# ajbrock/Neural-Photo-Editor

Hardware: NVIDIA H100
Metric: 64x64 images/sec IAN encode->decode @ batch 256 (higher is better)
Workload: dtype f32 (3-pass bf16 split on wgmma, fp32 accumulate)

## Files before the change

### neural-photo-editor_b200/csrc/ian_api.cu

```cuda
#include <cuda_runtime.h>

#include <algorithm>
#include <cmath>
#include <cstdarg>
#include <cstdio>
#include <cstdlib>
#include <cstring>
#include <map>
#include <string>
#include <vector>

#include <cuda.h>

#include "../../include/ian_b200.h"
#include "edge.h"
#include "tapgemm.h"

using namespace ian;

namespace {

thread_local std::string g_create_error;

inline uint16_t f2bf(float f) {
// ... 133 lines not shown
                                    "jvp_full_dec_fc2", "jvp_full_dec_conv1", "jvp_dec_conv2a", "jvp_dec_conv2a2", "jvp_full_dec_conv2",
                                    "jvp_dec_conv3a", "jvp_dec_conv3a2", "jvp_full_dec_conv3", "jvp_dec_conv4a", "jvp_dec_conv4a2",
                                    "jvp_full_dec_conv4", "rgb_head_jvp",
                                    "jvp_enc_conv2", "jvp_enc_conv3", "jvp_enc_conv4", "jvp_enc_fc1", "jvp_enc_head",
                                    "enc_conv1", "dec_out", "brush_seed", "enc_conv1_bwd",
                                    "wgrad_l_dec_fc2", "wgrad_dec_conv1", "wgrad_dec_conv2", "wgrad_dec_conv3", "wgrad_dec_out",
                                    "dec_out_jvp", "jvp_enc_conv1"};

struct DevWeights {
  __nv_bfloat16* b = nullptr;
  long long plane = 0;
  int ntiles = 0, Cout = 0, Cin = 0;
  float* scale = nullptr;
  float* shift = nullptr;
};

struct Plan;

}

struct ian_handle {
  int device = 0;
  int model_kind = 0;
  int path = IAN_PATH_TC;
  int passes = 3;
  float* sk_ws = nullptr;
  int* sk_flags = nullptr;
  int sk_epoch = 0;
  int streamk = 1;
  bool splitk = true;
  bool coop_finalize = true;
  bool pdl = true;
  bool graphs = true;
  bool capturing = false;
  bool finalized = false;
  cudaStream_t stream = nullptr;
  cudaStream_t h2d_stream = nullptr, d2h_stream = nullptr;
  std::vector<void*> host_allocs;
  int gw = 0, grank = 0, gn = 0, gcur = 0, gepoch = 0;
  float* gbuf = nullptr;
  float* gpeer_buf[8] = {nullptr};
  bool gconnected = false;
  float** gather_dsts = nullptr;
  int gather_ndst = 0;
  cudaStream_t push_stream = nullptr;
  cudaEvent_t g_comp[2] = {nullptr, nullptr}, g_done[2] = {nullptr, nullptr};
  bool g_done_valid[2] = {false, false};
  int g_last = -1;
  int push_ctas = 32;
  int push_mode = 0;
  void* train_ws = nullptr;
  size_t train_ws_bytes = 0;
  long long tickets = 0;
  struct Ticket { int id = -1, n = 0, slot = 0; };
  Ticket inflight[2];
  std::string err;
  int64_t launches = 0;
  std::map<std::string, HostParam> params;
  DevWeights w[L_COUNT];
  float* conv1_wt = nullptr;
  float* conv1_b = nullptr;
  __nv_bfloat16* conv1_tc_wt = nullptr;
  Conv1Maps* conv1_maps = nullptr;
  float* decout_wt = nullptr;
  float* conv1_bwd_wt = nullptr;
  __nv_bfloat16* conv1_bwd_tc_wt = nullptr;
// ... 480 lines not shown
int get_plan(ian_handle* h, int n, Plan** out) {
  auto it = h->plans.find(n);
  if (it != h->plans.end()) { *out = it->second; return IAN_OK; }
  Plan* pl = nullptr;
  int rc = build_plan(h, n, &pl);
  if (rc != IAN_OK) { if (pl) free_plan(pl); return rc; }
  h->plans[n] = pl;
  *out = pl;
  return IAN_OK;
}

struct ScopedTimer {
  ian_handle* h; int slot; cudaStream_t st; ian_handle::Timed tm{}; bool on;
  ScopedTimer(ian_handle* h_, int slot_, cudaStream_t st_) : h(h_), slot(slot_), st(st_), on(h_->timing) {
    if (on) { cudaEventCreate(&tm.e0); cudaEventCreate(&tm.e1); cudaEventRecord(tm.e0, st); }
  }
  ~ScopedTimer() {
    if (on) { cudaEventRecord(tm.e1, st); h->timed[slot].push_back(tm); }
  }
};

constexpr int kGraphMaxBatch = 32;

int run_gemm(ian_handle* h, Plan* pl, int l, cudaStream_t st) {
  TapGemm g = pl->g[l];
  if (g.ksplit < 1) return fail(h, IAN_ERR_INVALID, "layer %s is not part of this plan", kLayerNames[l]);
  g.passes = h->passes;
  g.out_t_bf16 = (g.out_f32_t && h->passes == 1) ? 1 : 0;
  const bool sk_ok = !h->capturing && (h->streamk == 2 || pl->n > kGraphMaxBatch);
  g.sk_ws = (h->streamk && sk_ok) ? h->sk_ws : nullptr;
  g.sk_force = h->streamk == 2 ? 1 : 0;
  g.sk_flags = h->sk_flags;
  g.sk_epoch = ++h->sk_epoch;
  ian_handle::Timed tm{};
  if (h->timing) {
    CUDA_TRY(h, cudaEventCreate(&tm.e0));
    CUDA_TRY(h, cudaEventCreate(&tm.e1));
  }
  if (h->path == IAN_PATH_SIMT) {
    g.ksplit = 1;
    g.ws = nullptr;
    if (h->timing) CUDA_TRY(h, cudaEventRecord(tm.e0, st));
    LAUNCH_TRY(h, launch_tapgemm_simt(g, st));
    if (h->timing) CUDA_TRY(h, cudaEventRecord(tm.e1, st));
  } else {
    if (h->timing) CUDA_TRY(h, cudaEventRecord(tm.e0, st));
    LAUNCH_TRY(h, launch_tapgemm_tc(g, pl->maps[l], st));
    if (h->timing) CUDA_TRY(h, cudaEventRecord(tm.e1, st));
    if (g.ksplit > 1) LAUNCH_TRY(h, launch_splitk_finalize(g, st));
  }
  if (h->timing) h->timed[l].push_back(tm);
  return IAN_OK;
}

int run_encode(ian_handle* h, Plan* pl, const float* x, const float* eps, float* z, cudaStream_t st, float* z_pre = nullptr) {
  const int n = pl->n;
  {
    ScopedTimer tm(h, T_CONV1, st);
    if (h->path == IAN_PATH_TC)
      LAUNCH_TRY(h, launch_conv1_tc(h->conv1_maps, pl->conv1_out, x, h->conv1_b, n, st));
    else
      LAUNCH_TRY(h, launch_conv1(x, h->conv1_wt, h->conv1_b, pl->a1.p, pl->a1.plane, n, st));
  }
  int rc;
  for (int l : kEncoder)
    if ((rc = run_gemm(h, pl, l, st)) != IAN_OK) return rc;
// ... 1333 lines not shown

extern "C" {

int ian_create(int model_kind, int device, ian_handle** out) {
  if (!out) return fail(nullptr, IAN_ERR_INVALID, "out is NULL");
  if (model_kind != IAN_MODEL_SIMPLE && model_kind != IAN_MODEL_FULL && model_kind != IAN_MODEL_V1)
    return fail(nullptr, IAN_ERR_UNSUPPORTED, "unknown model kind %d", model_kind);
  int ndev = 0;
  cudaError_t e = cudaGetDeviceCount(&ndev);
  if (e != cudaSuccess || ndev == 0)
    return fail(nullptr, IAN_ERR_CUDA, "no CUDA device: %s (this library has no CPU path)", cudaGetErrorString(e));
  if (device < 0 || device >= ndev) return fail(nullptr, IAN_ERR_INVALID, "device %d out of range [0,%d)", device, ndev);
  cudaDeviceProp prop;
  cudaGetDeviceProperties(&prop, device);
  if (prop.major != 9 || prop.minor != 0)
    return fail(nullptr, IAN_ERR_UNSUPPORTED, "device %d is sm_%d%d; libian_b200 is built for sm_90a only", device, prop.major, prop.minor);
  ian_handle* h = new ian_handle();
  h->device = device;
  h->model_kind = model_kind;
  DeviceGuard dg(device);
  if (cudaStreamCreateWithFlags(&h->stream, cudaStreamNonBlocking) != cudaSuccess ||
      cudaStreamCreateWithFlags(&h->h2d_stream, cudaStreamNonBlocking) != cudaSuccess ||
      cudaStreamCreateWithFlags(&h->d2h_stream, cudaStreamNonBlocking) != cudaSuccess) {
    delete h;
    return fail(nullptr, IAN_ERR_CUDA, "cudaStreamCreate failed");
  }
  if (const char* c = getenv("IAN_CHUNK")) { int v = atoi(c); if (v > 0) h->max_chunk = v > 4096 ? 4096 : v; }
  if (const char* c = getenv("IAN_PATH")) { if (!strcmp(c, "simt")) h->path = IAN_PATH_SIMT; }
  if (const char* c = getenv("IAN_STREAMK")) { const int v = atoi(c); h->streamk = v < 0 ? 0 : v > 2 ? 2 : v; }
  if (const char* c = getenv("IAN_SPLITK")) h->splitk = atoi(c) != 0;
  if (const char* c = getenv("IAN_PDL")) h->pdl = atoi(c) != 0;
  if (const char* c = getenv("IAN_FINALIZE8")) h->coop_finalize = atoi(c) != 0;
  if (const char* c = getenv("IAN_GRAPHS")) h->graphs = atoi(c) != 0;
  *out = h;
  return IAN_OK;
}

int ian_set_param(ian_handle* h, const char* name, const float* data, const int64_t* shape, int ndim) {
  if (!h || !name || !data || !shape) return fail(h, IAN_ERR_INVALID, "NULL argument");
  if (h->finalized) return fail(h, IAN_ERR_STATE, "model already finalized");
  int64_t elems = 0;
  int rc = check_param_shape(h, name, shape, ndim, &elems);
  if (rc != IAN_OK) return rc;
  HostParam& p = h->params[name];
  p.shape.assign(shape, shape + ndim);
  p.data.assign(data, data + elems);
  return IAN_OK;
}

int ian_set_made_ordering(ian_handle* h, const int32_t* ordering, int n) {
  if (!h || !ordering) return fail(h, IAN_ERR_INVALID, "NULL argument");
  if (h->finalized) return fail(h, IAN_ERR_STATE, "model already finalized");
  if (n != 100) return fail(h, IAN_ERR_INVALID, "ordering must have 100 entries (got %d)", n);
  std::vector<char> seen(100, 0);
  for (int i = 0; i < n; ++i) {
    if (ordering[i] < 0 || ordering[i] >= 100 || seen[ordering[i]]) return fail(h, IAN_ERR_INVALID, "ordering is not a permutation of 0..99");
    seen[ordering[i]] = 1;
  }
  h->made_ordering.assign(ordering, ordering + n);
  return IAN_OK;
}

int ian_model_param_count(int model_kind) {
  if (model_kind < 0 || model_kind > 2) return IAN_ERR_INVALID;
  return (int)cached_specs(model_kind).size();
}
// ... 574 lines not shown
```

### neural-photo-editor_b200/csrc/tapgemm.h

```cpp
#pragma once
#include <cuda_bf16.h>
#include <cuda_runtime.h>
#include <stdint.h>

#include <atomic>

namespace ian {

enum Act : int { ACT_NONE = 0, ACT_LRELU = 1, ACT_RELU = 2, ACT_ELU = 3, ACT_MASK = 4 };

constexpr int kMaxDevices = 64;
inline int cur_device() {
  int d = 0;
  cudaGetDevice(&d);
  return (d >= 0 && d < kMaxDevices) ? d : 0;
}
struct DeviceOnce {
  std::atomic<bool> done[kMaxDevices];
  bool is_done(int dev) const { return done[dev].load(std::memory_order_acquire); }
  void set_done(int dev) { done[dev].store(true, std::memory_order_release); }
};

inline bool& pdl_flag() {
  static thread_local bool on = false;
// ... 44 lines not shown
  int Hg, Wg;
  const __nv_bfloat16* b;
  long long b_plane;
  int Cout;
  int nphase;
  Phase phase[kMaxPhases];
  Tap taps[kMaxTaps];
  const float* scale;
  const float* shift;
  int scale_pix_stride;
  int act;
  const __nv_bfloat16* mask;
  float mask_slope;
  int res_after;
  __nv_bfloat16* out;
  long long out_plane;
  float* out_f32;
  int Hout, Wout, osh, osw;
  int ksplit;
  float* ws;
  long long ws_slab;
  const __nv_bfloat16* res;
  long long res_plane;
  __nv_bfloat16* out_raw;
  long long out_raw_plane;
  float* out_f32_t;
  int cout_real;
  int out_t_bf16;
  int passes;
  float* sk_ws;
  int* sk_flags;
  int sk_epoch;
  int sk_force;
};

__host__ __device__ inline void tile_shape(int Hg, int Wg, int& Wt, int& Ht, int& Nt) {
  Wt = Wg < 128 ? Wg : 128;
  Ht = Hg < 128 / Wt ? Hg : 128 / Wt;
  Nt = 128 / (Wt * Ht);
}

__device__ __forceinline__ float act_apply(float v, int act) {
  switch (act) {
    case ACT_LRELU: return 0.6f * v + 0.4f * fabsf(v);
    case ACT_RELU:  return 0.5f * (v + fabsf(v));
    case ACT_ELU:   return v > 0.f ? v : expm1f(v);
    default:        return v;
  }
}

__device__ __forceinline__ void split_bf16(float v, __nv_bfloat16& hi, __nv_bfloat16& lo) {
  hi = __float2bfloat16_rn(v);
  lo = __float2bfloat16_rn(v - __bfloat162float(hi));
}

int launch_tapgemm_simt(const TapGemm& g, cudaStream_t st);
struct TcMaps;
TcMaps* tc_build_maps(const TapGemm& g, char* err, int errlen);
void tc_free_maps(TcMaps*);
int launch_tapgemm_tc(const TapGemm& g, const TcMaps* maps, cudaStream_t st);
int launch_splitk_finalize(const TapGemm& g, cudaStream_t st);
int tc_tile_width(const TcMaps* maps);
int tc_num_sms();
size_t tc_sk_workspace_floats();
size_t tc_sk_flag_ints();

// ... 21 lines not shown
```

### neural-photo-editor_b200/csrc/tapgemm_tc.cu

```cuda
#include <cuda.h>

#include <cstdio>
#include <cstring>
#include <vector>

#include "tapgemm.h"
#include "tc_ptx.cuh"

namespace ian {

struct TcMaps {
  CUtensorMap a[4];
  CUtensorMap b;
  CUtensorMap a1[4];
  CUtensorMap b1;
  int Wt, Ht, Nt, BN;
  mutable int sk_choice;
};

namespace {

using namespace tc;

constexpr int BM = 128;
constexpr int BK = 64;

constexpr int kEpiWarps = 8;
constexpr int kThreadsCta = 32 * kEpiWarps + 32;

template <int BN, int PASSES> struct TcCfg {
  static constexpr int kPlanes = PASSES == 3 ? 2 : 1;
  static constexpr int kATileBytes = BM * BK * 2 * kPlanes;
  static constexpr int kBTileBytes = BN * BK * 2 * kPlanes;
  static constexpr int kStageBytes = kATileBytes + kBTileBytes;
  static constexpr int kRound = (PASSES == 3 && BN > 32) ? 32 : BN;
  static constexpr int kRounds = BN / kRound;
  static constexpr int kLd = kRound + 8;
  static constexpr int kStagingBytes = BM * kLd * 4;
  static constexpr int kStageSmem = kEpiWarps * 1024;
  static constexpr int kStagesFit = (220 * 1024 - kStagingBytes - kStageSmem) / kStageBytes;
  static constexpr int kStages = kStagesFit > 6 ? 6 : kStagesFit;
  static constexpr int kSmemBytes = kStages * kStageBytes + 1024  + 256  + kStageSmem + kStagingBytes;
  static_assert(kStages >= 2 && kSmemBytes <= 232448, "tapgemm_tc: shared memory budget");
};
static_assert(TcCfg<128, 3>::kStages == 3 && TcCfg<128, 3>::kSmemBytes == 226560, "tapgemm_tc: three float32-mode stages");

struct WorkItem {
  int phase, ks, co0, it0, it1;
  int n0, p0, q0, mtile;
  int sk_role, sk_last;
};

template <int CH, int PASSES>
__device__ __forceinline__ void store_split(__nv_bfloat16* dst, long long plane, const float (&v)[CH]) {
  __align__(16) __nv_bfloat162 hi[CH / 2], lo[CH / 2];
#pragma unroll
  for (int j = 0; j < CH / 2; ++j) {
    hi[j] = __floats2bfloat162_rn(v[2 * j], v[2 * j + 1]);
    if (PASSES == 3) {
      const float2 hf = __bfloat1622float2(hi[j]);
      lo[j] = __floats2bfloat162_rn(v[2 * j] - hf.x, v[2 * j + 1] - hf.y);
    }
  }
  static_assert(CH % 16 == 0, "an epilogue chunk is a whole number of 32-byte sectors per plane");
  const uint4* h4 = reinterpret_cast<const uint4*>(hi);
  const uint4* l4 = reinterpret_cast<const uint4*>(lo);
#pragma unroll
  for (int j = 0; j < CH / 16; ++j) {
    tc::st_global_256(dst + 16 * j, h4[2 * j], h4[2 * j + 1]);
    if (PASSES == 3) tc::st_global_256(dst + plane + 16 * j, l4[2 * j], l4[2 * j + 1]);
  }
}

template <int BN>
__device__ __forceinline__ WorkItem decode_work(const TapGemm& g, const TcMaps& maps, int w) {
  WorkItem wi;
  const int tiles_q = g.Wg / maps.Wt, tiles_p = g.Hg / maps.Ht;
  const int tiles_m = tiles_q * tiles_p * ((g.n_img + maps.Nt - 1) / maps.Nt);
// ... 42 lines not shown
      wi.sk_role = 0; wi.sk_last = 0;
      w += stride;
      return true;
    }
    if (cur >= end) return false;
    int gi = cur, ph = 0, phase_start = 0;
    while (ph + 1 < g.nphase && gi >= phase_start + tiles_per_phase * iters[ph]) { phase_start += tiles_per_phase * iters[ph]; ++ph; }
    const int ip = iters[ph];
    const int tile = (gi - phase_start) / ip, it = (gi - phase_start) % ip;
    int len = ip - it;
    if (len > end - gi) len = end - gi;
    wi.phase = ph; wi.ks = 0; wi.it0 = it; wi.it1 = it + len;
    int mt = tile % tiles_m;
    const int nt = tile / tiles_m;
    wi.mtile = mt;
    const int qb = mt % tiles_q; mt /= tiles_q;
    const int pb = mt % tiles_p; mt /= tiles_p;
    wi.n0 = mt * maps.Nt; wi.p0 = pb * maps.Ht; wi.q0 = qb * maps.Wt; wi.co0 = nt * BN;
    wi.sk_role = it > 0 ? 1 : (len < ip ? 2 : 0);
    wi.sk_last = wi.sk_role == 2 ? owner(phase_start + tile * ip + ip - 1) : 0;
    cur = gi + len;
    return true;
  }
};

template <int BN, int PASSES, bool SK>
__global__ void __launch_bounds__(kThreadsCta, 1)
tapgemm_tc_kernel(const __grid_constant__ TapGemm g, const __grid_constant__ TcMaps maps, const int total_work) {
  using Cfg = TcCfg<BN, PASSES>;
  constexpr int kATileBytes = Cfg::kATileBytes;
  constexpr int S = Cfg::kStages;
  extern __shared__ uint8_t smem_raw[];
  const uint32_t smem_base = (smem_u32(smem_raw) + 1023u) & ~1023u;
  const uint32_t bar_base = smem_base + S * Cfg::kStageBytes;
  auto full_bar = [&](int s) { return bar_base + 8u * s; };
  auto empty_bar = [&](int s) { return bar_base + 8u * (S + s); };
  const uint32_t stage_smem = bar_base + 256u;
  uint8_t* smem_al = smem_raw + (smem_base - smem_u32(smem_raw));
  float* stage_ptr = reinterpret_cast<float*>(smem_al + (stage_smem - smem_base));
  float* acc_tile = stage_ptr + kEpiWarps * 256;

  const int warp = threadIdx.x >> 5, lane = threadIdx.x & 31;

  if (threadIdx.x == 0) {
    pdl_trigger();
    for (int s = 0; s < S; ++s) {
      mbar_init(full_bar(s), 1);
      mbar_init(empty_bar(s), 2);
    }
    asm volatile("fence.mbarrier_init.release.cluster;" ::: "memory");
  }
  __syncthreads();
  pdl_wait();

  if (warp == kEpiWarps) {
    uint32_t i = 0;
    WorkIter<BN, SK> iter;
    iter.init(g, maps, total_work);
    WorkItem wi;
    while (iter.next(g, maps, wi)) {
      const Phase ph = g.phase[wi.phase];
      int t = wi.it0 % ph.ntaps, c0 = wi.it0 / ph.ntaps * BK;
      for (int it = wi.it0; it < wi.it1; ++it, ++i) {
        const int s = i % S;
        const uint32_t par = (i / S) & 1u;
        const Tap tap = g.taps[ph.tap_begin + t];
        mbar_wait(empty_bar(s), par ^ 1u);
        const uint32_t sa = smem_base + s * Cfg::kStageBytes;
        if (elect_one_sync()) {
          mbar_expect_tx(full_bar(s), Cfg::kStageBytes);
          tma_load_5d(PASSES == 3 ? &maps.a[tap.view] : &maps.a1[tap.view], full_bar(s), sa, c0, wi.q0 + tap.dw,
                      wi.p0 + tap.dh, wi.n0, 0);
          tma_load_3d(PASSES == 3 ? &maps.b : &maps.b1, full_bar(s), sa + kATileBytes, c0, tap.wtile * g.Cout + wi.co0, 0);
        }
        __syncwarp();
        if (++t == ph.ntaps) { t = 0; c0 += BK; }
      }
    }
    return;
  }

  constexpr int R = BN / 2;
  constexpr int RW = Cfg::kRound;
  constexpr int TC = RW >= 32 ? RW / 2 : RW;
  constexpr int CH = TC >= 32 ? 32 : 16;
  constexpr int kThreadCols = Cfg::kRounds * TC;
  const int wg = warp >> 2, wtid = threadIdx.x & 127;
  const int ew = warp;
  const int lg = warp & 3;
  const int half = ew >> 2;
  const bool has_cols = RW >= 32 || half == 0;
  float* my_stage = stage_ptr + ew * 256;
  const float act_a = g.act == ACT_LRELU ? 0.6f : g.act == ACT_RELU ? 0.5f : 1.f;
  const float act_b = g.act == ACT_LRELU ? 0.4f : g.act == ACT_RELU ? 0.5f : 0.f;
  const int ml = lg * 32 + lane;
  const int wl = ml % maps.Wt;
  const int hl = (ml / maps.Wt) % maps.Ht;
  const int nl = ml / (maps.Wt * maps.Ht);
  uint32_t i = 0;
  WorkIter<BN, SK> iter;
  iter.init(g, maps, total_work);
  WorkItem wi;
  while (iter.next(g, maps, wi)) {
    const Phase ph = g.phase[wi.phase];
    if (wi.it1 <= wi.it0) continue;
    if (has_cols && g.scale_pix_stride == 0) {
      __syncwarp();
      for (int c = lane; c < BN; c += 32) {
        my_stage[c] = g.scale ? __ldg(g.scale + wi.co0 + c) : 1.f;
        my_stage[128 + c] = g.shift ? __ldg(g.shift + wi.co0 + c) : 0.f;
      }
      __syncwarp();
    }
    float acc_m[R], acc_c[PASSES == 3 ? R : 1];
#pragma unroll
    for (int j = 0; j < R; ++j) acc_m[j] = 0.f;
#pragma unroll
    for (int j = 0; j < (PASSES == 3 ? R : 1); ++j) acc_c[j] = 0.f;
    wgmma_fence_regs(acc_m);
    if (PASSES == 3) wgmma_fence_regs(acc_c);
    for (int it = wi.it0; it < wi.it1; ++it, ++i) {
      const int s = i % S;
      mbar_wait(full_bar(s), (i / S) & 1u);
      const uint32_t sa = smem_base + s * Cfg::kStageBytes;
      const uint64_t a_hi = make_sw128_desc(sa + wg * 64 * 128), a_lo = make_sw128_desc(sa + BM * BK * 2 + wg * 64 * 128);
      const uint64_t b_hi = make_sw128_desc(sa + kATileBytes), b_lo = make_sw128_desc(sa + kATileBytes + BN * BK * 2);
      const uint32_t first = (it == wi.it0) ? 0u : 1u;
      wgmma_fence();
#pragma unroll
      for (int k = 0; k < BK / 16; ++k) {
        const uint64_t ko = (uint64_t)(k * 2);
        const uint32_t acc = k > 0 ? 1u : first;
        wgmma_bf16<BN>(acc_m, a_hi + ko, b_hi + ko, acc);
        if constexpr (PASSES == 3) {
          wgmma_bf16<BN>(acc_c, a_lo + ko, b_hi + ko, acc);
          wgmma_bf16<BN>(acc_c, a_hi + ko, b_lo + ko, 1u);
        }
      }
      wgmma_commit();
      wgmma_wait<1>();
      if (it > wi.it0 && wtid == 0) mbar_arrive(empty_bar((i - 1) % S));
    }
    wgmma_wait<0>();
    wgmma_fence_regs(acc_m);
    if (PASSES == 3) wgmma_fence_regs(acc_c);
    if (wtid == 0) mbar_arrive(empty_bar((i - 1) % S));
    if constexpr (PASSES == 3) {
#pragma unroll
      for (int j = 0; j < R; ++j) acc_m[j] += acc_c[j];
    }
    if (SK && wi.sk_role == 2 && has_cols) {
      for (int k = (int)blockIdx.x + 1 + lane; k <= wi.sk_last; k += 32) {
        if (iter.boundary(k) == iter.boundary(k + 1)) continue;
        const int* fl = g.sk_flags + k * kEpiWarps + ew;
        const long long t0 = clock64();
        int fv;
        do {
          asm volatile("ld.acquire.gpu.global.s32 %0, [%1];" : "=r"(fv) : "l"(fl) : "memory");
          if (clock64() - t0 > 4000000000LL) __trap();
        } while (fv != g.sk_epoch);
      }
      __syncwarp();
    }
    const int n = wi.n0 + nl, p = wi.p0 + hl, q = wi.q0 + wl;
    const bool valid = n < g.n_img;
    const int oh = p * g.osh + ph.oh0, ow = q * g.osw + ph.ow0;
    const long long pix = (long long)(n * g.Hout + oh) * g.Wout + ow;
#pragma unroll 1
    for (int r = 0; r < Cfg::kRounds; ++r) {
      asm volatile("bar.sync 1, 256;" ::: "memory");
#pragma unroll
      for (int j = 0; j < RW / 2; j += 2) {
        float2 v = make_float2(acc_m[j], acc_m[j + 1]);
#pragma unroll
        for (int rr = 1; rr < Cfg::kRounds; ++rr)
          if (rr == r) v = make_float2(acc_m[rr * RW / 2 + j], acc_m[rr * RW / 2 + j + 1]);
        *reinterpret_cast<float2*>(acc_tile + (wg * 64 + frag_row(wtid, j)) * Cfg::kLd + frag_col(wtid, j)) = v;
      }
      asm volatile("bar.sync 1, 256;" ::: "memory");
      if (!has_cols) continue;
#pragma unroll 1
      for (int cc = 0; cc < TC; cc += CH) {
        const int cb = r * RW + half * TC + cc;
        const int co = wi.co0 + cb;
        const int cs = r * TC + cc;
        float v[CH];
        const float* srow = acc_tile + ml * Cfg::kLd + half * TC + cc;
#pragma unroll
        for (int j = 0; j < CH / 4; ++j) {
          const float4 t4 = *reinterpret_cast<const float4*>(srow + 4 * j);
          v[4 * j] = t4.x; v[4 * j + 1] = t4.y; v[4 * j + 2] = t4.z; v[4 * j + 3] = t4.w;
        }
        if (SK && wi.sk_role == 1) {
          float4* wp = reinterpret_cast<float4*>(g.sk_ws + (((long long)blockIdx.x * kEpiWarps + ew) * 32 + lane) * kThreadCols + cs);
#pragma unroll
          for (int j = 0; j < CH / 4; ++j) __stcg(wp + j, make_float4(v[4 * j], v[4 * j + 1], v[4 * j + 2], v[4 * j + 3]));
// ... 89 lines not shown
            }
          }
          if (g.out) store_split<CH, PASSES>(g.out + off, g.out_plane, v);
          if (g.out_f32_t) {
            const long long tbase = ((long long)wi.mtile * g.cout_real + co) * BM + ml;
            if (g.out_t_bf16) {
              __nv_bfloat16* ot = reinterpret_cast<__nv_bfloat16*>(g.out_f32_t) + tbase;
#pragma unroll
              for (int j = 0; j < CH; ++j)
                if (co + j < g.cout_real) ot[j * BM] = __float2bfloat16_rn(v[j]);
            } else {
              float* ot = g.out_f32_t + tbase;
#pragma unroll
              for (int j = 0; j < CH; ++j)
                if (co + j < g.cout_real) ot[j * BM] = v[j];
            }
          }
          if (g.out_f32) {
            float4* of = reinterpret_cast<float4*>(g.out_f32 + off);
#pragma unroll
            for (int j = 0; j < CH / 4; ++j) of[j] = make_float4(v[4 * j], v[4 * j + 1], v[4 * j + 2], v[4 * j + 3]);
          }
        }
      }
    }
    if (SK && wi.sk_role == 1 && has_cols) {
      __threadfence();
      __syncwarp();
      if (lane == 0) {
        int* fl = g.sk_flags + (int)blockIdx.x * kEpiWarps + ew;
        asm volatile("st.release.gpu.global.s32 [%0], %1;" ::"l"(fl), "r"(g.sk_epoch) : "memory");
      }
    }
  }
}

}

TcMaps* tc_build_maps(const TapGemm& g, char* err, int errlen) {
  tc::EncodeTiledFn enc = tc::get_encode_fn();
  if (!enc) { snprintf(err, errlen, "cuTensorMapEncodeTiled entry point not available"); return nullptr; }
  if (g.Cin % 64 || (g.Cout % 128 && g.Cout != 16)) { snprintf(err, errlen, "tc path needs Cin%%64==0 and Cout%%128==0 or Cout==16 (got %d,%d)", g.Cin, g.Cout); return nullptr; }
  TcMaps* m = new TcMaps();
  memset(m, 0, sizeof(*m));
  tile_shape(g.Hg, g.Wg, m->Wt, m->Ht, m->Nt);
  m->sk_choice = -1;
  m->BN = (g.Cout % 128 == 0) ? 128 : 16;
  if (g.Wg % m->Wt || g.Hg % m->Ht || m->Wt * m->Ht * m->Nt != BM) {
    snprintf(err, errlen, "M grid %dx%d does not tile into 128-row boxes", g.Hg, g.Wg);
    delete m; return nullptr;
  }
  bool used[4] = {false, false, false, false};
  int max_tile = 0;
  for (int p = 0; p < g.nphase; ++p)
    for (int t = 0; t < g.phase[p].ntaps; ++t) {
      const Tap& tp = g.taps[g.phase[p].tap_begin + t];
      used[tp.view] = true;
      if (tp.wtile > max_tile) max_tile = tp.wtile;
    }
  for (int v = 0; v < 4; ++v) {
    if (!used[v]) continue;
    const int vh = v >> 1, vw = v & 1;
    const cuuint64_t Hv = (g.Hin - vh + g.sh - 1) / g.sh, Wv = (g.Win - vw + g.sw - 1) / g.sw;
    cuuint64_t dims[5] = {(cuuint64_t)g.Cin, Wv, Hv, (cuuint64_t)g.n_img, 2};
    cuuint64_t strides[4] = {(cuuint64_t)g.sw * g.Cin * 2, (cuuint64_t)g.sh * g.Win * g.Cin * 2,
                             (cuuint64_t)g.Hin * g.Win * g.Cin * 2, (cuuint64_t)g.a_plane * 2};
    cuuint32_t box[5] = {BK, (cuuint32_t)m->Wt, (cuuint32_t)m->Ht, (cuuint32_t)m->Nt, 2};
    cuuint32_t estr[5] = {1, 1, 1, 1, 1};
    void* base = (void*)(g.a + ((long long)vh * g.Win + vw) * g.Cin);
    CUresult r = enc(&m->a[v], CU_TENSOR_MAP_DATA_TYPE_BFLOAT16, 5, base, dims, strides, box, estr,
                     CU_TENSOR_MAP_INTERLEAVE_NONE, CU_TENSOR_MAP_SWIZZLE_128B, CU_TENSOR_MAP_L2_PROMOTION_L2_256B,
                     CU_TENSOR_MAP_FLOAT_OOB_FILL_NONE);
    if (r != CUDA_SUCCESS) { snprintf(err, errlen, "cuTensorMapEncodeTiled(A view %d) failed: %d", v, (int)r); delete m; return nullptr; }
    box[4] = 1;
    r = enc(&m->a1[v], CU_TENSOR_MAP_DATA_TYPE_BFLOAT16, 5, base, dims, strides, box, estr, CU_TENSOR_MAP_INTERLEAVE_NONE,
            CU_TENSOR_MAP_SWIZZLE_128B, CU_TENSOR_MAP_L2_PROMOTION_L2_256B, CU_TENSOR_MAP_FLOAT_OOB_FILL_NONE);
    if (r != CUDA_SUCCESS) { snprintf(err, errlen, "cuTensorMapEncodeTiled(A1 view %d) failed: %d", v, (int)r); delete m; return nullptr; }
  }
  {
    cuuint64_t dims[3] = {(cuuint64_t)g.Cin, (cuuint64_t)(max_tile + 1) * g.Cout, 2};
    cuuint64_t strides[2] = {(cuuint64_t)g.Cin * 2, (cuuint64_t)g.b_plane * 2};
    cuuint32_t box[3] = {BK, (cuuint32_t)m->BN, 2};
    cuuint32_t estr[3] = {1, 1, 1};
    CUresult r = enc(&m->b, CU_TENSOR_MAP_DATA_TYPE_BFLOAT16, 3, (void*)g.b, dims, strides, box, estr,
                     CU_TENSOR_MAP_INTERLEAVE_NONE, CU_TENSOR_MAP_SWIZZLE_128B, CU_TENSOR_MAP_L2_PROMOTION_L2_256B,
                     CU_TENSOR_MAP_FLOAT_OOB_FILL_NONE);
    if (r != CUDA_SUCCESS) { snprintf(err, errlen, "cuTensorMapEncodeTiled(B) failed: %d", (int)r); delete m; return nullptr; }
    box[2] = 1;
    r = enc(&m->b1, CU_TENSOR_MAP_DATA_TYPE_BFLOAT16, 3, (void*)g.b, dims, strides, box, estr, CU_TENSOR_MAP_INTERLEAVE_NONE,
            CU_TENSOR_MAP_SWIZZLE_128B, CU_TENSOR_MAP_L2_PROMOTION_L2_256B, CU_TENSOR_MAP_FLOAT_OOB_FILL_NONE);
    if (r != CUDA_SUCCESS) { snprintf(err, errlen, "cuTensorMapEncodeTiled(B1) failed: %d", (int)r); delete m; return nullptr; }
  }
  return m;
}

void tc_free_maps(TcMaps* m) { delete m; }

int tc_tile_width(const TcMaps* maps) { return maps->BN; }

int tc_num_sms() {
  static std::atomic<int> num_sms[kMaxDevices];
  const int dev = cur_device();
  int n = num_sms[dev].load(std::memory_order_relaxed);
  if (!n) {
    cudaDeviceGetAttribute(&n, cudaDevAttrMultiProcessorCount, dev);
    num_sms[dev].store(n, std::memory_order_relaxed);
  }
  return n;
}
size_t tc_sk_workspace_floats() { return (size_t)tc_num_sms() * kEpiWarps * 32 * 128; }
size_t tc_sk_flag_ints() { return (size_t)tc_num_sms() * kEpiWarps; }

template <int BN, int PASSES, bool SK>
static int launch_one(const TapGemm& g, const TcMaps* maps, int tiles_m, int num_sms, cudaStream_t st) {
  using Cfg = TcCfg<BN, PASSES>;
  static DeviceOnce attr_set;
  const int dev = cur_device();
  if (!attr_set.is_done(dev)) {
    if (cudaFuncSetAttribute(tapgemm_tc_kernel<BN, PASSES, SK>, cudaFuncAttributeMaxDynamicSharedMemorySize, Cfg::kSmemBytes) != cudaSuccess)
      return -1;
    attr_set.set_done(dev);
  }
  int total_work, grid;
  if (SK) {
    long long T = 0;
    for (int p = 0; p < g.nphase; ++p) T += (long long)tiles_m * (g.Cout / maps->BN) * g.phase[p].ntaps * (g.Cin / BK);
    total_work = (int)T;
    grid = num_sms;
  } else {
    total_work = tiles_m * (g.Cout / maps->BN) * g.nphase * g.ksplit;
    grid = total_work < num_sms ? total_work : num_sms;
  }
  if (launch_pdl(tapgemm_tc_kernel<BN, PASSES, SK>, dim3(grid), dim3(kThreadsCta), Cfg::kSmemBytes, st, g, *maps, total_work) != cudaSuccess)
    return -1;
  return cudaGetLastError() == cudaSuccess ? 1 : -1;
}

int launch_tapgemm_tc(const TapGemm& g, const TcMaps* maps, cudaStream_t st) {
  const int num_sms = tc_num_sms();
  const int tiles_m = (g.Wg / maps->Wt) * (g.Hg / maps->Ht) * ((g.n_img + maps->Nt - 1) / maps->Nt);
  const long long tiles = (long long)tiles_m * (g.Cout / maps->BN) * g.nphase;
  bool sk = false;
  if (g.sk_force) {
    sk = g.sk_ws && g.ksplit == 1 && maps->BN == 128 && !g.out_f32_t;
  } else if (maps->sk_choice >= 0) {
    sk = maps->sk_choice == 1 && g.sk_ws != nullptr;
  } else if (g.sk_ws && g.ksplit == 1 && maps->BN == 128 && tiles >= num_sms / 2 && !g.out_f32_t) {
    const int per_phase = tiles_m * (g.Cout / maps->BN);
    std::vector<long long> load(num_sms, 0);
    long long T = 0;
    for (long long w = 0; w < tiles; ++w) {
      const int it = g.phase[w / per_phase].ntaps * (g.Cin / BK);
      load[w % num_sms] += it;
      T += it;
    }
    long long makespan = 0;
    for (long long v : load) makespan = v > makespan ? v : makespan;
    sk = makespan * num_sms >= (T * 6) / 5;
    maps->sk_choice = sk ? 1 : 0;
  } else if (g.sk_ws) {
    maps->sk_choice = 0;
  }
  if (g.passes == 1) {
    if (maps->BN == 128) return sk ? launch_one<128, 1, true>(g, maps, tiles_m, num_sms, st) : launch_one<128, 1, false>(g, maps, tiles_m, num_sms, st);
    return launch_one<16, 1, false>(g, maps, tiles_m, num_sms, st);
  }
  if (maps->BN == 128) return sk ? launch_one<128, 3, true>(g, maps, tiles_m, num_sms, st) : launch_one<128, 3, false>(g, maps, tiles_m, num_sms, st);
  return launch_one<16, 3, false>(g, maps, tiles_m, num_sms, st);
}

}
// ... 1 lines not shown
```

### neural-photo-editor_b200/csrc/tc_ptx.cuh

```cuda
#pragma once
#include <cuda.h>
#include <stdint.h>

namespace ian {
namespace tc {

__device__ __forceinline__ uint32_t smem_u32(const void* p) { return (uint32_t)__cvta_generic_to_shared(p); }

__device__ __forceinline__ bool elect_one_sync() {
  uint32_t pred;
  asm volatile(
      "{\n\t.reg .pred P1;\n\t"
      "elect.sync _|P1, 0xffffffff;\n\t"
      "selp.b32 %0, 1, 0, P1;\n\t}"
      : "=r"(pred));
  return pred != 0;
}

__device__ __forceinline__ void st_global_256(void* p, const uint4& a, const uint4& b) {
  asm volatile("st.global.v4.b32 [%0], {%1, %2, %3, %4};" ::"l"(p), "r"(a.x), "r"(a.y), "r"(a.z), "r"(a.w) : "memory");
  asm volatile("st.global.v4.b32 [%0], {%1, %2, %3, %4};" ::"l"(reinterpret_cast<uint8_t*>(p) + 16), "r"(b.x), "r"(b.y),
               "r"(b.z), "r"(b.w)
               : "memory");
}
// ... 15 lines not shown
      "selp.u32 %0, 1, 0, p;\n\t}"
      : "=r"(ok)
      : "r"(bar), "r"(parity)
      : "memory");
  return ok != 0;
}
__device__ __forceinline__ void mbar_wait(uint32_t bar, uint32_t parity) {
  if (mbar_try_wait(bar, parity)) return;
  const long long t0 = clock64();
  while (!mbar_try_wait(bar, parity)) {
    if (clock64() - t0 > 4000000000LL) __trap();
  }
}

__device__ __forceinline__ void tma_load_5d(const CUtensorMap* map, uint32_t bar, uint32_t dst, int c0, int c1, int c2,
                                            int c3, int c4) {
  asm volatile(
      "cp.async.bulk.tensor.5d.shared::cluster.global.mbarrier::complete_tx::bytes [%0], [%1, {%3, %4, %5, %6, %7}], [%2];"
      ::"r"(dst), "l"(map), "r"(bar), "r"(c0), "r"(c1), "r"(c2), "r"(c3), "r"(c4)
      : "memory");
}
__device__ __forceinline__ void tma_load_3d(const CUtensorMap* map, uint32_t bar, uint32_t dst, int c0, int c1, int c2) {
  asm volatile(
      "cp.async.bulk.tensor.3d.shared::cluster.global.mbarrier::complete_tx::bytes [%0], [%1, {%3, %4, %5}], [%2];"
      ::"r"(dst), "l"(map), "r"(bar), "r"(c0), "r"(c1), "r"(c2)
      : "memory");
}

__device__ __forceinline__ void tma_store_3d(const CUtensorMap* map, uint32_t src, int c0, int c1, int c2) {
  asm volatile("cp.async.bulk.tensor.3d.global.shared::cta.bulk_group [%0, {%2, %3, %4}], [%1];" ::"l"(map), "r"(src), "r"(c0),
               "r"(c1), "r"(c2)
               : "memory");
}
__device__ __forceinline__ void bulk_commit_group() { asm volatile("cp.async.bulk.commit_group;" ::: "memory"); }
__device__ __forceinline__ void bulk_wait_group_read0() { asm volatile("cp.async.bulk.wait_group.read 0;" ::: "memory"); }
__device__ __forceinline__ void bulk_wait_group0() { asm volatile("cp.async.bulk.wait_group 0;" ::: "memory"); }
__device__ __forceinline__ void fence_proxy_async_smem() { asm volatile("fence.proxy.async.shared::cta;" ::: "memory"); }
__device__ __forceinline__ void st_shared_v4(uint32_t addr, const uint4& v) {
  asm volatile("st.shared.v4.b32 [%0], {%1, %2, %3, %4};" ::"r"(addr), "r"(v.x), "r"(v.y), "r"(v.z), "r"(v.w) : "memory");
}

__device__ __forceinline__ void wgmma_fence() { asm volatile("wgmma.fence.sync.aligned;" ::: "memory"); }
__device__ __forceinline__ void wgmma_commit() { asm volatile("wgmma.commit_group.sync.aligned;" ::: "memory"); }
template <int N> __device__ __forceinline__ void wgmma_wait() { asm volatile("wgmma.wait_group.sync.aligned %0;" ::"n"(N) : "memory"); }
template <int R> __device__ __forceinline__ void wgmma_fence_regs(float (&d)[R]) {
#pragma unroll
  for (int j = 0; j < R; ++j) asm volatile("" : "+f"(d[j])::"memory");
}

template <int N> __device__ __forceinline__ void wgmma_bf16(float (&d)[N / 2], uint64_t a, uint64_t b, uint32_t accum);
template <> __device__ __forceinline__ void wgmma_bf16<16>(float (&d)[8], uint64_t a, uint64_t b, uint32_t accum) {
  asm volatile(
      "{\n\t.reg .pred p;\n\t"
      "setp.ne.b32 p, %10, 0;\n\t"
      "wgmma.mma_async.sync.aligned.m64n16k16.f32.bf16.bf16 "
      "{%0, %1, %2, %3, %4, %5, %6, %7}, %8, %9, p, 1, 1, 0, 0;\n\t}"
      : "+f"(d[0]), "+f"(d[1]), "+f"(d[2]), "+f"(d[3]), "+f"(d[4]), "+f"(d[5]), "+f"(d[6]), "+f"(d[7])
      : "l"(a), "l"(b), "r"(accum));
}
template <> __device__ __forceinline__ void wgmma_bf16<40>(float (&d)[20], uint64_t a, uint64_t b, uint32_t accum) {
  asm volatile(
      "{\n\t.reg .pred p;\n\t"
      "setp.ne.b32 p, %22, 0;\n\t"
      "wgmma.mma_async.sync.aligned.m64n40k16.f32.bf16.bf16 "
      "{%0, %1, %2, %3, %4, %5, %6, %7, %8, %9, %10, %11, %12, %13, %14, %15, %16, %17, %18, %19}, %20, %21, p, 1, 1, 0, 0;\n\t}"
      : "+f"(d[0]), "+f"(d[1]), "+f"(d[2]), "+f"(d[3]), "+f"(d[4]), "+f"(d[5]), "+f"(d[6]), "+f"(d[7]), "+f"(d[8]), "+f"(d[9]), "+f"(d[10]), "+f"(d[11]), "+f"(d[12]), "+f"(d[13]), "+f"(d[14]), "+f"(d[15]), "+f"(d[16]), "+f"(d[17]), "+f"(d[18]), "+f"(d[19])
      : "l"(a), "l"(b), "r"(accum));
}
// ... 80 lines not shown
```

Baseline: 82720.

## Add TMA-store epilogue for 3-pass BN=128 tapgemm output

Adds an epilogue path for the 3-pass, BN=128, non-split-K case. It applies scale/shift and the activation, splits each result into bf16 hi/lo planes in swizzled shared staging buffers, and writes them with 5D TMA bulk tensor stores. Two double-buffered rounds let the async stores overlap with the next round of register-to-smem writes. The path is meant to cut per-thread global store overhead, but it reshapes the shared-memory budget, adds named barriers across the epilogue warps, and falls back to the old path for residual, mask and f32 outputs.

Result: faster. 86790, median of 6 (+4.9%).

```diff
diff --git a/neural-photo-editor_b200/csrc/ian_api.cu b/neural-photo-editor_b200/csrc/ian_api.cu
--- a/neural-photo-editor_b200/csrc/ian_api.cu
+++ b/neural-photo-editor_b200/csrc/ian_api.cu
@@ -189,6 +189,7 @@
   bool coop_finalize = true;
   bool pdl = true;
   bool graphs = true;
+  bool epi_tma = true;
   bool capturing = false;
   bool finalized = false;
   cudaStream_t stream = nullptr;
@@ -735,6 +736,7 @@
   g.sk_force = h->streamk == 2 ? 1 : 0;
   g.sk_flags = h->sk_flags;
   g.sk_epoch = ++h->sk_epoch;
+  g.epi_tma = h->epi_tma ? 1 : 0;
   ian_handle::Timed tm{};
   if (h->timing) {
     CUDA_TRY(h, cudaEventCreate(&tm.e0));
@@ -2134,6 +2136,7 @@
   if (const char* c = getenv("IAN_PDL")) h->pdl = atoi(c) != 0;
   if (const char* c = getenv("IAN_FINALIZE8")) h->coop_finalize = atoi(c) != 0;
   if (const char* c = getenv("IAN_GRAPHS")) h->graphs = atoi(c) != 0;
+  if (const char* c = getenv("IAN_EPI_TMA")) h->epi_tma = atoi(c) != 0;
   *out = h;
   return IAN_OK;
 }
diff --git a/neural-photo-editor_b200/csrc/tapgemm.h b/neural-photo-editor_b200/csrc/tapgemm.h
--- a/neural-photo-editor_b200/csrc/tapgemm.h
+++ b/neural-photo-editor_b200/csrc/tapgemm.h
@@ -100,6 +100,7 @@
   int* sk_flags;
   int sk_epoch;
   int sk_force;
+  int epi_tma;
 };
 
 __host__ __device__ inline void tile_shape(int Hg, int Wg, int& Wt, int& Ht, int& Nt) {
diff --git a/neural-photo-editor_b200/csrc/tapgemm_tc.cu b/neural-photo-editor_b200/csrc/tapgemm_tc.cu
--- a/neural-photo-editor_b200/csrc/tapgemm_tc.cu
+++ b/neural-photo-editor_b200/csrc/tapgemm_tc.cu
@@ -14,6 +14,9 @@
   CUtensorMap b;
   CUtensorMap a1[4];
   CUtensorMap b1;
+  CUtensorMap o[2];
+  const __nv_bfloat16* o_out;
+  long long o_plane;
   int Wt, Ht, Nt, BN;
   mutable int sk_choice;
 };
@@ -36,14 +39,18 @@
   static constexpr int kRound = (PASSES == 3 && BN > 32) ? 32 : BN;
   static constexpr int kRounds = BN / kRound;
   static constexpr int kLd = kRound + 8;
-  static constexpr int kStagingBytes = BM * kLd * 4;
-  static constexpr int kStageSmem = kEpiWarps * 1024;
-  static constexpr int kStagesFit = (220 * 1024 - kStagingBytes - kStageSmem) / kStageBytes;
+  static constexpr bool kTmaEpi = PASSES == 3 && BN == 128;
+  static constexpr int kOutPlaneBytes = BM * kRound * 2;
+  static constexpr int kOutRoundBytes = 2 * kOutPlaneBytes;
+  static constexpr int kStagingBytes = kTmaEpi && 2 * kOutRoundBytes > BM * kLd * 4 ? 2 * kOutRoundBytes : BM * kLd * 4;
+  static constexpr int kStageSmem = kTmaEpi ? 1024 : kEpiWarps * 1024;
+  static constexpr int kStagesFit = (232448 - 1024 - 256 - kStagingBytes - kStageSmem) / kStageBytes;
   static constexpr int kStages = kStagesFit > 6 ? 6 : kStagesFit;
   static constexpr int kSmemBytes = kStages * kStageBytes + 1024  + 256  + kStageSmem + kStagingBytes;
   static_assert(kStages >= 2 && kSmemBytes <= 232448, "tapgemm_tc: shared memory budget");
 };
-static_assert(TcCfg<128, 3>::kStages == 3 && TcCfg<128, 3>::kSmemBytes == 226560, "tapgemm_tc: three float32-mode stages");
+static_assert(TcCfg<128, 3>::kStages == 3 && TcCfg<128, 3>::kSmemBytes == 231680, "tapgemm_tc: three float32-mode stages");
+static_assert(TcCfg<128, 3>::kRound == 32 && TcCfg<128, 3>::kOutRoundBytes == 16384, "tapgemm_tc: 32-column TMA-store rounds");
 
 struct WorkItem {
   int phase, ks, co0, it0, it1;
@@ -152,13 +159,14 @@
   constexpr int S = Cfg::kStages;
   extern __shared__ uint8_t smem_raw[];
   const uint32_t smem_base = (smem_u32(smem_raw) + 1023u) & ~1023u;
-  const uint32_t bar_base = smem_base + S * Cfg::kStageBytes;
+  const uint32_t stg_base = smem_base + S * Cfg::kStageBytes;
+  const uint32_t bar_base = stg_base + Cfg::kStagingBytes;
   auto full_bar = [&](int s) { return bar_base + 8u * s; };
   auto empty_bar = [&](int s) { return bar_base + 8u * (S + s); };
   const uint32_t stage_smem = bar_base + 256u;
   uint8_t* smem_al = smem_raw + (smem_base - smem_u32(smem_raw));
   float* stage_ptr = reinterpret_cast<float*>(smem_al + (stage_smem - smem_base));
-  float* acc_tile = stage_ptr + kEpiWarps * 256;
+  float* acc_tile = reinterpret_cast<float*>(smem_al + (stg_base - smem_base));
 
   const int warp = threadIdx.x >> 5, lane = threadIdx.x & 31;
 
@@ -210,13 +218,13 @@
   const int lg = warp & 3;
   const int half = ew >> 2;
   const bool has_cols = RW >= 32 || half == 0;
-  float* my_stage = stage_ptr + ew * 256;
+  float* my_stage = stage_ptr + (Cfg::kTmaEpi ? 0 : ew * 256);
   const float act_a = g.act == ACT_LRELU ? 0.6f : g.act == ACT_RELU ? 0.5f : 1.f;
   const float act_b = g.act == ACT_LRELU ? 0.4f : g.act == ACT_RELU ? 0.5f : 0.f;
   const int ml = lg * 32 + lane;
-  const int wl = ml % maps.Wt;
-  const int hl = (ml / maps.Wt) % maps.Ht;
-  const int nl = ml / (maps.Wt * maps.Ht);
+  const int wl0 = ml % maps.Wt;
+  const int hl0 = (ml / maps.Wt) % maps.Ht;
+  const int nl0 = ml / (maps.Wt * maps.Ht);
   uint32_t i = 0;
   WorkIter<BN, SK> iter;
   iter.init(g, maps, total_work);
@@ -224,13 +232,21 @@
   while (iter.next(g, maps, wi)) {
     const Phase ph = g.phase[wi.phase];
     if (wi.it1 <= wi.it0) continue;
-    if (has_cols && g.scale_pix_stride == 0) {
-      __syncwarp();
-      for (int c = lane; c < BN; c += 32) {
-        my_stage[c] = g.scale ? __ldg(g.scale + wi.co0 + c) : 1.f;
-        my_stage[128 + c] = g.shift ? __ldg(g.shift + wi.co0 + c) : 0.f;
-      }
-      __syncwarp();
+    if (g.scale_pix_stride == 0) {
+      if constexpr (Cfg::kTmaEpi) {
+        asm volatile("bar.sync 1, 256;" ::: "memory");
+        for (int c = threadIdx.x; c < BN; c += 32 * kEpiWarps) {
+          my_stage[c] = g.scale ? __ldg(g.scale + wi.co0 + c) : 1.f;
+          my_stage[128 + c] = g.shift ? __ldg(g.shift + wi.co0 + c) : 0.f;
+        }
+      } else if (has_cols) {
+        __syncwarp();
+        for (int c = lane; c < BN; c += 32) {
+          my_stage[c] = g.scale ? __ldg(g.scale + wi.co0 + c) : 1.f;
+          my_stage[128 + c] = g.shift ? __ldg(g.shift + wi.co0 + c) : 0.f;
+        }
+        __syncwarp();
+      }
     }
     float acc_m[R], acc_c[PASSES == 3 ? R : 1];
 #pragma unroll
@@ -269,6 +285,49 @@
 #pragma unroll
       for (int j = 0; j < R; ++j) acc_m[j] += acc_c[j];
     }
+    if constexpr (Cfg::kTmaEpi) {
+      if (g.epi_tma && wi.sk_role == 0) {
+#pragma unroll
+        for (int r = 0; r < Cfg::kRounds; ++r) {
+          const uint32_t buf = stg_base + (uint32_t)(r & 1) * Cfg::kOutRoundBytes;
+          if (threadIdx.x == 0) bulk_wait_group_read1();
+          asm volatile("bar.sync 1, 256;" ::: "memory");
+#pragma unroll
+          for (int j = 0; j < RW / 2; j += 2) {
+            const float2 a = make_float2(acc_m[r * RW / 2 + j], acc_m[r * RW / 2 + j + 1]);
+            const int row = wg * 64 + frag_row(wtid, j);
+            const int c = frag_col(wtid, j);
+            const float2 sc = *reinterpret_cast<const float2*>(my_stage + r * RW + c);
+            const float2 sf = *reinterpret_cast<const float2*>(my_stage + 128 + r * RW + c);
+            float v0 = fmaf(a.x, sc.x, sf.x), v1 = fmaf(a.y, sc.y, sf.y);
+            if (g.act == ACT_ELU) {
+              v0 = v0 > 0.f ? v0 : expm1f(v0);
+              v1 = v1 > 0.f ? v1 : expm1f(v1);
+            } else if (g.act != ACT_NONE) {
+              v0 = fmaf(act_b, fabsf(v0), act_a * v0);
+              v1 = fmaf(act_b, fabsf(v1), act_a * v1);
+            }
+            const __nv_bfloat162 hi = __floats2bfloat162_rn(v0, v1);
+            const float2 hf = __bfloat1622float2(hi);
+            const __nv_bfloat162 lo = __floats2bfloat162_rn(v0 - hf.x, v1 - hf.y);
+            const uint32_t off = (uint32_t)row * 64u + ((((uint32_t)c >> 3) ^ (((uint32_t)row >> 1) & 3u)) << 4) + ((uint32_t)c & 7u) * 2u;
+            asm volatile("st.shared.b32 [%0], %1;" ::"r"(buf + off), "r"(*reinterpret_cast<const uint32_t*>(&hi)) : "memory");
+            asm volatile("st.shared.b32 [%0], %1;" ::"r"(buf + Cfg::kOutPlaneBytes + off), "r"(*reinterpret_cast<const uint32_t*>(&lo))
+                         : "memory");
+          }
+          fence_proxy_async_smem();
+          asm volatile("bar.sync 1, 256;" ::: "memory");
+          if (threadIdx.x == 0) {
+            const int c4 = wi.n0 * g.Hg + wi.p0;
+            tma_store_5d(&maps.o[0], buf, wi.co0 + r * RW, ph.ow0, wi.q0, ph.oh0, c4);
+            tma_store_5d(&maps.o[1], buf + Cfg::kOutPlaneBytes, wi.co0 + r * RW, ph.ow0, wi.q0, ph.oh0, c4);
+            bulk_commit_group();
+          }
+        }
+        continue;
+      }
+      if (threadIdx.x == 0) bulk_wait_group_read0();
+    }
     if (SK && wi.sk_role == 2 && has_cols) {
       for (int k = (int)blockIdx.x + 1 + lane; k <= wi.sk_last; k += 32) {
         if (iter.boundary(k) == iter.boundary(k + 1)) continue;
@@ -282,6 +341,15 @@
       }
       __syncwarp();
     }
+    int nl = nl0, hl = hl0, wl = wl0;
+    if constexpr (SK && Cfg::kTmaEpi) {
+      uint32_t tid;
+      asm volatile("mov.u32 %0, %%tid.x;" : "=r"(tid));
+      const int row = (int)((tid >> 5) & 3u) * 32 + (int)(tid & 31u);
+      wl = row % maps.Wt;
+      hl = (row / maps.Wt) % maps.Ht;
+      nl = row / (maps.Wt * maps.Ht);
+    }
     const int n = wi.n0 + nl, p = wi.p0 + hl, q = wi.q0 + wl;
     const bool valid = n < g.n_img;
     const int oh = p * g.osh + ph.oh0, ow = q * g.osw + ph.ow0;
@@ -437,6 +505,9 @@
         asm volatile("st.release.gpu.global.s32 [%0], %1;" ::"l"(fl), "r"(g.sk_epoch) : "memory");
       }
     }
+  }
+  if constexpr (Cfg::kTmaEpi) {
+    if (threadIdx.x == 0) bulk_wait_group0();
   }
 }
 
@@ -496,6 +567,20 @@
             CU_TENSOR_MAP_SWIZZLE_128B, CU_TENSOR_MAP_L2_PROMOTION_L2_256B, CU_TENSOR_MAP_FLOAT_OOB_FILL_NONE);
     if (r != CUDA_SUCCESS) { snprintf(err, errlen, "cuTensorMapEncodeTiled(B1) failed: %d", (int)r); delete m; return nullptr; }
   }
+  if (g.out && m->BN == 128 && g.Hout == g.osh * g.Hg && g.Wout == g.osw * g.Wg && (g.out_plane * 2) % 16 == 0 &&
+      (uintptr_t)g.out % 16 == 0) {
+    const cuuint64_t C = (cuuint64_t)g.Cout;
+    cuuint64_t dims[5] = {C, (cuuint64_t)g.osw, (cuuint64_t)g.Wg, (cuuint64_t)g.osh, (cuuint64_t)g.n_img * g.Hg};
+    cuuint64_t strides[4] = {C * 2, C * 2 * g.osw, C * 2 * g.Wout, C * 2 * g.Wout * g.osh};
+    cuuint32_t box[5] = {32, 1, (cuuint32_t)m->Wt, 1, (cuuint32_t)(m->Ht * m->Nt)};
+    cuuint32_t estr[5] = {1, 1, 1, 1, 1};
+    bool ok = true;
+    for (int pl = 0; pl < 2 && ok; ++pl)
+      ok = enc(&m->o[pl], CU_TENSOR_MAP_DATA_TYPE_BFLOAT16, 5, (void*)(g.out + pl * g.out_plane), dims, strides, box, estr,
+               CU_TENSOR_MAP_INTERLEAVE_NONE, CU_TENSOR_MAP_SWIZZLE_64B, CU_TENSOR_MAP_L2_PROMOTION_NONE,
+               CU_TENSOR_MAP_FLOAT_OOB_FILL_NONE) == CUDA_SUCCESS;
+    if (ok) { m->o_out = g.out; m->o_plane = g.out_plane; }
+  }
   return m;
 }
 
@@ -541,7 +626,12 @@
   return cudaGetLastError() == cudaSuccess ? 1 : -1;
 }
 
-int launch_tapgemm_tc(const TapGemm& g, const TcMaps* maps, cudaStream_t st) {
+int launch_tapgemm_tc(const TapGemm& g_in, const TcMaps* maps, cudaStream_t st) {
+  TapGemm g = g_in;
+  g.epi_tma = g_in.epi_tma && g.passes == 3 && maps->BN == 128 && g.ksplit == 1 && g.out && g.out == maps->o_out &&
+              g.out_plane == maps->o_plane && g.scale_pix_stride == 0 &&
+              (g.act == ACT_NONE || g.act == ACT_LRELU || g.act == ACT_RELU || g.act == ACT_ELU) && !g.out_raw && !g.res &&
+              !g.mask && !g.out_f32 && !g.out_f32_t;
   const int num_sms = tc_num_sms();
   const int tiles_m = (g.Wg / maps->Wt) * (g.Hg / maps->Ht) * ((g.n_img + maps->Nt - 1) / maps->Nt);
   const long long tiles = (long long)tiles_m * (g.Cout / maps->BN) * g.nphase;
diff --git a/neural-photo-editor_b200/csrc/tc_ptx.cuh b/neural-photo-editor_b200/csrc/tc_ptx.cuh
--- a/neural-photo-editor_b200/csrc/tc_ptx.cuh
+++ b/neural-photo-editor_b200/csrc/tc_ptx.cuh
@@ -71,8 +71,14 @@
                "r"(c1), "r"(c2)
                : "memory");
 }
+__device__ __forceinline__ void tma_store_5d(const CUtensorMap* map, uint32_t src, int c0, int c1, int c2, int c3, int c4) {
+  asm volatile("cp.async.bulk.tensor.5d.global.shared::cta.bulk_group [%0, {%2, %3, %4, %5, %6}], [%1];" ::"l"(map), "r"(src),
+               "r"(c0), "r"(c1), "r"(c2), "r"(c3), "r"(c4)
+               : "memory");
+}
 __device__ __forceinline__ void bulk_commit_group() { asm volatile("cp.async.bulk.commit_group;" ::: "memory"); }
 __device__ __forceinline__ void bulk_wait_group_read0() { asm volatile("cp.async.bulk.wait_group.read 0;" ::: "memory"); }
+__device__ __forceinline__ void bulk_wait_group_read1() { asm volatile("cp.async.bulk.wait_group.read 1;" ::: "memory"); }
 __device__ __forceinline__ void bulk_wait_group0() { asm volatile("cp.async.bulk.wait_group 0;" ::: "memory"); }
 __device__ __forceinline__ void fence_proxy_async_smem() { asm volatile("fence.proxy.async.shared::cta;" ::: "memory"); }
 __device__ __forceinline__ void st_shared_v4(uint32_t addr, const uint4& v) {
```
